# YushenLi807/WWW24-RAT

Hardware: AMD Instinct MI355X
Metric: training samples/sec at B=4096, K=10 retrieved, d=64; 1/2/4/8 MI355X (higher is better)
Workload: dtype f32; 1 GPU; synthetic_F20_V1M_K10_d64_B4096; fields=20, vocab_rows=1000000, retrieved=10, embedding_dim=64, batch_per_gpu=4096, global_batch=4096, heads=8, dim_head=10, depth=4, scale_dim=2, step=fwd+bwd+clip+adam, embedding_grad=atomic, sync_batch_norm=False, parallelism=dp1

## Files before the change

www24-rat_amd/csrc/attn.hip:

```cpp
#include "rat_device.h"
#include "../../include/rat_hip.h"

#include <cstdlib>
#include <initializer_list>

namespace {

constexpr int ATT_THREADS = 512;
constexpr int ATT_WAVES = ATT_THREADS / 64;
constexpr int ATT_ROWS = 64;
constexpr int ATT_MT = ATT_ROWS / 16;
constexpr int DH_MAX = 16;
constexpr int QSLOTS = 8;
constexpr int OSLOTS = 4;
constexpr int FAST_INNER = 80;
constexpr int fast_heads(int tdh) { return tdh > 0 ? FAST_INNER / tdh : 0; }
constexpr int CORE_UNROLL = 3;

struct AttnArgs {
    const float* x;
    const float* dy;
    float* y;
    const float* res;
    const float* add;
// ... 996 lines not shown
    RAT_REQUIRE(d <= 128, "embedding_dim > 128 is not supported by this kernel");
    RAT_REQUIRE(map->L >= 1 && map->L <= ATT_ROWS, "sequence length (K+1 or F+1) must be in [1, 64]");
    RAT_REQUIRE(map->nseq >= 1 && map->q_div >= 1, "bad seq map");
    const AttnGeom g(d, heads, dim_head);
    RAT_REQUIRE(g.fwd_smem() <= 160 * 1024, "heads*dim_head too large for the LDS tile (forward)");
    if (backward) {
        RAT_REQUIRE(g.bwd_smem(heads) <= 160 * 1024, "heads*dim_head too large for the LDS tile (backward)");
        RAT_REQUIRE((g.Q16 / 16) * (g.D16 / 16) <= QSLOTS * ATT_WAVES,
                    "3*heads*dim_head x embedding_dim exceeds the in-register dW_qkv accumulator budget");
        RAT_REQUIRE((g.D16 / 16) * (g.I16 / 16) <= OSLOTS * ATT_WAVES,
                    "embedding_dim x heads*dim_head exceeds the in-register dW_out accumulator budget");
    }
    return 0;
}

bool aligned16(const void* p) { return (reinterpret_cast<uintptr_t>(p) & 15) == 0; }

void fill_common(AttnArgs& a, const RatAttnParams* w, const RatSeqMap* map, int d, int heads, int dim_head,
                 float ln_eps) {
    a.ln_g = w->ln_g;
    a.ln_b = w->ln_b;
    a.w_qkv = w->w_qkv;
    a.w_out = w->w_out;
    a.b_out = w->b_out;
    a.nseq = map->nseq;
    a.q_div = map->q_div;
    a.hi_stride = map->hi_stride;
    a.lo_stride = map->lo_stride;
    a.pos_stride = map->pos_stride;
    a.L = map->L;
    a.nq = (map->queries > 0 && map->queries < map->L) ? map->queries : map->L;
    a.nsq_chunk = ATT_ROWS / map->L;
    a.nchunks = (map->nseq + a.nsq_chunk - 1) / a.nsq_chunk;
    a.d = d;
    a.heads = heads;
    a.dh = dim_head;
    a.eps = ln_eps;
    a.scale = 1.0f / sqrtf((float)dim_head);
    a.out_scale = 1.0f;
    const int I = heads * dim_head;
    a.vec_wqkv = (d % 4 == 0) && aligned16(w->w_qkv);
    a.vec_wout = (I % 4 == 0) && aligned16(w->w_out);
    a.prof = rat_prof_buffer();
}

bool aligned8(const void* p) { return (reinterpret_cast<uintptr_t>(p) & 7) == 0; }

int fast_dim(const AttnArgs& a, std::initializer_list<const void*> ptrs) {
    if (!((a.dh == 10 || a.dh == 20) && a.heads == fast_heads(a.dh)) || a.w_out == nullptr) return 0;
    for (const void* p : ptrs)
        if (p != nullptr && !aligned16(p)) return 0;
    if (!aligned16(a.w_qkv) || !aligned16(a.w_out)) return 0;
    return (a.d == 64 || a.d == 16) ? a.d : 0;
}

}

extern "C" int rat_attn_fwd(const float* x, float* y, float* o_save, float* lse_save, const RatAttnParams* w_host,
                            const RatSeqMap* map_host, int d, int heads, int dim_head, float ln_eps, void* stream) {
    return rat_attn_fwd_ex(x, x, y, o_save, lse_save, w_host, map_host, d, heads, dim_head, 0.f, 1.f, ln_eps, 0.f, 0, RAT_ARITH_F32,
                           nullptr, 0, stream);
}

static bool b3_dim(int d) { return d == B3_D || d == 40 || d == 48 || d == 56; }
static bool b3_geom(int d, int heads, int dim_head) {
    return (b3_dim(d) && heads == B3_H && dim_head == B3_DH) || (d == B3_D && heads == 4 && dim_head == 2 * B3_DH);
}
static bool b3_shape(int d, int heads, int dim_head, const RatAttnParams* w) {
    return b3_geom(d, heads, dim_head) && w->w_out != nullptr;
}
static bool b3_ph_fits(int L, int nsq_chunk, int heads = B3_H) { return (size_t)nsq_chunk * heads * L * L * 4 <= (size_t)3 * B3_XP; }
static int b3_matrix_core(int L) {
    const int k = rat_knob(RAT_KNOB_ATTN_BWD_CORE_MFMA);
    if (L > 48 || k == 0) return 0;
    if (L > 32) return (k == 1 || L >= 40) ? 13 : 0;
    return (k == 1 || L >= 28) ? (L > 16 ? 2 : 1) : 0;
}
static int b3_fwd_matrix_core(int L, int nq) {
    const int k = rat_knob(RAT_KNOB_ATTN_FWD_CORE_MFMA);
    if (L > 48 || nq < L || k == 3) return 0;
    if (k != 2 && !((L >= 28 && L <= 32) || L >= 40)) return 0;
    return L > 32 ? 3 : (L > 16 ? 2 : 1);
}
static bool b3_ph_enabled() {
    return rat_knob(RAT_KNOB_ATTN_BWD_PH) != 0;
}
static int b3_nvalid(int d) { return d == B3_D ? 0 : d; }
static bool b3_off32_ok(const RatSeqMap* m) {
    if (m->hi_stride < 0 || m->lo_stride < 0 || m->pos_stride < 0) return false;
    const int64_t qd = m->q_div, hi = (m->nseq - 1) / qd, lo = m->nseq - 1 < qd - 1 ? m->nseq - 1 : qd - 1;
    const double max_tok = (double)hi * (double)m->hi_stride + (double)lo * (double)m->lo_stride + (double)(m->L - 1) * (double)m->pos_stride;
    return (max_tok + 1.0) * (double)(B3_I * 4) < 4294967296.0;
}

extern "C" size_t rat_attn_fwd_workspace(int d, int heads, int dim_head) {
    return b3_geom(d, heads, dim_head) ? B3_W_QKV + B3_W_OUT : 0;
}

extern "C" size_t rat_attn_planes_bytes(int d, int heads, int dim_head) {
    return b3_geom(d, heads, dim_head) ? B3_W_BYTES : 0;
}
extern "C" int rat_attn_split_jobs(const RatAttnParams* w_host, int d, int heads, int dim_head, void* planes, RatSplitJob* jobs_out) {
    RAT_REQUIRE(w_host && jobs_out, "null pointer");
    if (!b3_shape(d, heads, dim_head, w_host) || planes == nullptr) return 0;
    RAT_REQUIRE(aligned16(planes) && w_host->w_qkv, "planes must be 16-byte aligned");
    char* ws = static_cast<char*>(planes);
    jobs_out[0] = RatSplitJob{w_host->w_qkv, ws, B3_Q3, d, d, 0, 0, 0};
    jobs_out[1] = RatSplitJob{w_host->w_out, ws + B3_W_QKV, B3_I, d, B3_I, 1, 0, 0};
    jobs_out[2] = RatSplitJob{w_host->w_qkv, ws + B3_W_QKV + B3_W_OUTT, B3_D, B3_Q3, d, 1, 0, b3_nvalid(d)};
    jobs_out[3] = RatSplitJob{w_host->w_out, ws + B3_W_QKV + B3_W_OUTT + B3_W_QKVT, B3_D, B3_I, B3_I, 0, 0, b3_nvalid(d)};
    return 4;
}

extern "C" int rat_attn_fwd_ex(const float* x, const float* res, float* y, float* o_save, float* lse_save,
                               const RatAttnParams* w_host, const RatSeqMap* map_host, int d, int heads, int dim_head,
                               float softmax_scale, float out_scale, float ln_eps, float dropout_p, uint64_t dropout_seed,
                               int arith, float* workspace, size_t workspace_bytes, void* stream) {
    if (check_dims(map_host, d, heads, dim_head, false)) return -1;
    RAT_REQUIRE(x && y && w_host && w_host->ln_g && w_host->ln_b && w_host->w_qkv, "null pointer");
    RAT_REQUIRE(w_host->w_out != nullptr || heads * dim_head == d, "missing w_out");
    AttnArgs a{};
    fill_common(a, w_host, map_host, d, heads, dim_head, ln_eps);
    if (softmax_scale > 0.f) a.scale = softmax_scale;
    a.out_scale = out_scale;
    a.res = res;
    a.x = x;
    a.y = y;
    a.o_save = o_save;
    a.lse_save = lse_save;
    a.vec_x = (d % 4 == 0) && aligned16(x) && aligned16(y) && aligned16(res);
    const AttnGeom g(d, heads, dim_head);
    const bool ct_shape = dim_head == 10 && ((d == 10 && (heads == 8 || heads == 2)) || (d == 16 && heads == 2));
    const size_t smem = g.fwd_smem() + (ct_shape ? ct_weight_floats(g) * sizeof(float) : 0);
    const int per_cu = (int)((160 * 1024) / smem) >= 2 ? 2 : 1;
    const unsigned blocks = (unsigned)(a.nchunks < rat_max_blocks() * per_cu ? a.nchunks : rat_max_blocks() * per_cu);
    RAT_REQUIRE(dropout_p >= 0.f && dropout_p < 1.f, "dropout_p must be in [0, 1)");
    if (dropout_p > 0.f && w_host->w_out != nullptr)
        a.drop = RatDrop{dropout_seed, (uint32_t)((double)dropout_p * 4294967296.0), 1.0f / (1.0f - dropout_p), w_host->drop_seed_dev};
    const int fast = fast_dim(a, {x, y, res, o_save, lse_save});
    const bool plain = res == x && out_scale == 1.0f && a.drop.threshold == 0;
    const bool have_planes = w_host->planes != nullptr && aligned16(w_host->planes);
    const bool dpad = d != B3_D && b3_dim(d) && heads == fast_heads(dim_head) && aligned16(x) && aligned16(y) && aligned16(res) &&
                      aligned16(o_save) && aligned16(lse_save) && aligned16(w_host->w_qkv) && aligned16(w_host->w_out);
    if (arith == RAT_ARITH_BF16X3 && (fast == 64 || dpad) && b3_shape(d, heads, dim_head, w_host) && b3_off32_ok(map_host) &&
        (have_planes || (workspace != nullptr && workspace_bytes >= B3_W_QKV + B3_W_OUT && aligned16(workspace)))) {
        const char* p_qkv;
        const char* p_out;
        if (have_planes) {
            p_qkv = static_cast<const char*>(w_host->planes);
            p_out = p_qkv + B3_W_QKV + B3_W_OUTT + B3_W_QKVT;
        } else {
            char* ws = reinterpret_cast<char*>(workspace);
            if (rat_launch_split_weights(w_host->w_qkv, B3_Q3, d, d, 0, ws, stream) ||
                rat_launch_split_weights(w_host->w_out, B3_D, B3_I, B3_I, 0, ws + B3_W_QKV, stream, 0, b3_nvalid(d))) return -1;
            p_qkv = ws;
            p_out = ws + B3_W_QKV;
        }
        Attn3W W{};
        W.qkv = RatWPlanes{reinterpret_cast<const rat_u4*>(p_qkv), 2};
        W.out = RatWPlanes{reinterpret_cast<const rat_u4*>(p_out), 3};
        const unsigned b3_blocks = (unsigned)(a.nchunks < rat_max_blocks() ? a.nchunks : rat_max_blocks());
        if (heads == 4) {
            RAT_LAUNCH((attn_fwd3_kernel<true, false, false, false, 0, 4>), b3_blocks, ATT_THREADS, b3_fwd_smem(), stream, a, W);
            return rat_check_launch("rat_attn_fwd (bf16x3, 4 heads)");
        }
        if (dpad) {
            if (plain && a.nq < a.L) RAT_LAUNCH((attn_fwd3_kernel<false, true, true>), b3_blocks, ATT_THREADS, b3_fwd_smem(), stream, a, W);
            else if (plain) RAT_LAUNCH((attn_fwd3_kernel<false, false, true>), b3_blocks, ATT_THREADS, b3_fwd_smem(), stream, a, W);
            else RAT_LAUNCH((attn_fwd3_kernel<true, false, true>), b3_blocks, ATT_THREADS, b3_fwd_smem(), stream, a, W);
        } else if (plain && a.nq < a.L) RAT_LAUNCH((attn_fwd3_kernel<false, true>), b3_blocks, ATT_THREADS, b3_fwd_smem(), stream, a, W);
        else if (plain && b3_fwd_matrix_core(a.L, a.nq) == 3)
            RAT_LAUNCH((attn_fwd3_kernel<false, false, false, false, 3>), b3_blocks, ATT_THREADS, b3_fwd_smem(), stream, a, W);
        else if (plain && b3_fwd_matrix_core(a.L, a.nq) == 2)
            RAT_LAUNCH((attn_fwd3_kernel<false, false, false, false, 2>), b3_blocks, ATT_THREADS, b3_fwd_smem(), stream, a, W);
        else if (plain && b3_fwd_matrix_core(a.L, a.nq) == 1)
            RAT_LAUNCH((attn_fwd3_kernel<false, false, false, false, 1>), b3_blocks, ATT_THREADS, b3_fwd_smem(), stream, a, W);
        else if (plain) RAT_LAUNCH((attn_fwd3_kernel<false>), b3_blocks, ATT_THREADS, b3_fwd_smem(), stream, a, W);
        else if (b3_fwd_matrix_core(a.L, a.L) == 3)
            RAT_LAUNCH((attn_fwd3_kernel<true, false, false, false, 3>), b3_blocks, ATT_THREADS, b3_fwd_smem(), stream, a, W);
        else if (b3_fwd_matrix_core(a.L, a.L) == 2)
            RAT_LAUNCH((attn_fwd3_kernel<true, false, false, false, 2>), b3_blocks, ATT_THREADS, b3_fwd_smem(), stream, a, W);
        else RAT_LAUNCH((attn_fwd3_kernel<true>), b3_blocks, ATT_THREADS, b3_fwd_smem(), stream, a, W);
        return rat_check_launch("rat_attn_fwd (bf16x3)");
    }
    const bool head_vec = aligned8(o_save);
    RAT_REQUIRE(head_vec || dim_head <= DH_MAX, "o_save must be 8-byte aligned for dim_head 20");
    if (!head_vec) RAT_LAUNCH((attn_fwd_kernel<0, 0>), blocks, ATT_THREADS, smem, stream, a);
    else if (fast == 64 && dim_head == 10 && plain) RAT_LAUNCH((attn_fwd_kernel<64, 10, false>), blocks, ATT_THREADS, smem, stream, a);
    else if (fast == 64 && dim_head == 10) RAT_LAUNCH((attn_fwd_kernel<64, 10>), blocks, ATT_THREADS, smem, stream, a);
    else if (fast == 16 && dim_head == 10) RAT_LAUNCH((attn_fwd_kernel<16, 10>), blocks, ATT_THREADS, smem, stream, a);
    else if (fast == 64 && dim_head == 20) RAT_LAUNCH((attn_fwd_kernel<64, 20>), blocks, ATT_THREADS, smem, stream, a);
    else if (dim_head == 20) RAT_LAUNCH((attn_fwd_kernel<0, 20>), blocks, ATT_THREADS, smem, stream, a);
    else if (dim_head == 10 && d == 10 && heads == 8) RAT_LAUNCH((attn_fwd_kernel<0, 10, true, 2, 8, 10>), blocks, ATT_THREADS, smem, stream, a);
    else if (dim_head == 10 && d == 10 && heads == 2) RAT_LAUNCH((attn_fwd_kernel<0, 10, true, 2, 2, 10>), blocks, ATT_THREADS, smem, stream, a);
    else if (dim_head == 10 && d == 16 && heads == 2) RAT_LAUNCH((attn_fwd_kernel<0, 10, true, 2, 2, 16>), blocks, ATT_THREADS, smem, stream, a);
    else if (dim_head == 10 && d <= 16) RAT_LAUNCH((attn_fwd_kernel<0, 10, true, 2>), blocks, ATT_THREADS, smem, stream, a);
    else if (dim_head == 10) RAT_LAUNCH((attn_fwd_kernel<0, 10>), blocks, ATT_THREADS, smem, stream, a);
    else RAT_LAUNCH((attn_fwd_kernel<0, 0>), blocks, ATT_THREADS, smem, stream, a);
    return rat_check_launch("rat_attn_fwd");
}

static int b3_groups(int d, int heads, int dim_head) {
    return (d == B3_D && dim_head == B3_DH && heads > B3_H && heads % B3_H == 0 && heads / B3_H <= 8) ? heads / B3_H : 0;
}
static int wide_heads(int dim_head) { return dim_head == WG_DH ? WG_H : (dim_head == 2 * WG_DH ? WG_H / 2 : 0); }
static int wide_groups(int d, int heads, int dim_head) {
    const int wh = wide_heads(dim_head);
    return (d >= 1 && d <= 16 && wh > 0 && heads > wh && heads % wh == 0 && heads / wh <= 8) ? heads / wh : 0;
}
extern "C" int rat_attn_groups_supported(int d, int heads, int dim_head) {
    if (b3_groups(d, heads, dim_head)) return 1;
    const int G = wide_groups(d, heads, dim_head);
    return G == 0 ? 0 : (G <= WG_MAXG ? 3 : 1);
}
extern "C" size_t rat_attn_groups_planes_bytes(int d, int heads, int dim_head) {
    return (size_t)b3_groups(d, heads, dim_head) * B3_GRP_PLANES;
}
extern "C" int rat_attn_groups_split_jobs(const RatAttnParams* w_host, int d, int heads, int dim_head, void* planes, RatSplitJob* jobs_out) {
    RAT_REQUIRE(w_host && jobs_out, "null pointer");
    const int G = b3_groups(d, heads, dim_head);
    if (G == 0 || planes == nullptr || w_host->w_out == nullptr) return 0;
    RAT_REQUIRE(aligned16(planes) && w_host->w_qkv, "planes must be 16-byte aligned");
    const int I = heads * dim_head;
    int n = 0;
    const int rows = (B3_I << 8) | (I << 20);
    for (int g = 0; g < G; ++g) {
        char* ws = static_cast<char*>(planes) + (size_t)g * B3_GRP_PLANES;
        const float* wq = w_host->w_qkv + (size_t)g * B3_I * d;
        const float* wo = w_host->w_out + (size_t)g * B3_I;
        jobs_out[n++] = RatSplitJob{wq, ws, B3_Q3, d, d, 0, rows, 0};
        jobs_out[n++] = RatSplitJob{wo, ws + B3_W_QKV, B3_I, d, I, 1, 0, 0};
        jobs_out[n++] = RatSplitJob{wq, ws + B3_W_QKV + B3_W_OUTT, B3_D, B3_Q3, d, 1, rows, 0};
        jobs_out[n++] = RatSplitJob{wo, ws + B3_W_QKV + B3_W_OUTT + B3_W_QKVT, B3_D, B3_I, I, 0, 0, 0};
    }
    return n;
}
extern "C" int rat_attn_fwd_groups(const float* x, const float* res, float* y, float* o_save, float* lse_save, int64_t ntok,
                                   const RatAttnParams* w_host, const void* planes, const RatSeqMap* map_host, int d, int heads,
                                   int dim_head, float softmax_scale, float out_scale, float ln_eps, float dropout_p,
                                   uint64_t dropout_seed, void* stream) {
    const int Gw = wide_groups(d, heads, dim_head);
    if (Gw > 0) {
        const int wh = wide_heads(dim_head);
        if (check_dims(map_host, d, wh, dim_head, false)) return -1;
        RAT_REQUIRE(x && y && w_host && w_host->ln_g && w_host->ln_b && w_host->w_qkv && w_host->w_out && w_host->b_out, "null pointer");
        RAT_REQUIRE((o_save == nullptr) == (lse_save == nullptr) && ntok > 0, "o_save and lse_save come together, [G][ntok][.]");
        AttnArgs a{};
        fill_common(a, w_host, map_host, d, wh, dim_head, ln_eps);
        a.vec_wout = ((heads * dim_head) % 4 == 0) && aligned16(w_host->w_out);
        a.vec_wqkv = (aligned8(x) && aligned16(w_host->w_out)) ? 1 : 0;
        if (softmax_scale > 0.f) a.scale = softmax_scale;
        a.out_scale = out_scale;
        a.res = res;
        a.x = x;
        a.y = y;
        a.o_save = o_save;
        a.lse_save = lse_save;
        a.groups = Gw;
        a.group_tok = ntok;
// ... 219 lines not shown
```

www24-rat_amd/csrc/attn_b3.h:

```cpp
constexpr int B3_D = 64, B3_I = 80, B3_Q3 = 240, B3_H = 8, B3_DH = 10;
constexpr int B3_LDQ = B3_Q3 + 4;
constexpr int B3_XP = 64 * 128;
constexpr int B3_OP = 64 * 160 + 64;
constexpr int B3_QP = 64 * 480;
typedef RatPlanes<128, 7, B3_XP> PlanesX;
typedef RatPlanes<160, 0, B3_OP> PlanesO;
typedef RatPlanes<480, 0, B3_QP> PlanesQ;

struct Attn3W {
    RatWPlanes qkv;
    RatWPlanes out;
    RatWPlanes outT;
    RatWPlanes qkvT;
};
constexpr size_t B3_W_QKV = (size_t)15 * 2 * 3 * 1024, B3_W_OUT = (size_t)4 * 3 * 3 * 1024, B3_W_OUTT = (size_t)5 * 2 * 3 * 1024,
                 B3_W_QKVT = (size_t)4 * 8 * 3 * 1024;
constexpr size_t B3_W_BYTES = B3_W_QKV + B3_W_OUT + B3_W_OUTT + B3_W_QKVT;

constexpr size_t B3_FWD_LSE = (size_t)3 * B3_XP + (size_t)64 * B3_LDQ * 4 + (size_t)3 * B3_OP + 2 * 64 * 8;
constexpr size_t B3_FWD_WOUT = B3_FWD_LSE + (size_t)64 * B3_H * 4;
constexpr size_t b3_fwd_smem() { return B3_FWD_WOUT + B3_W_OUT; }
constexpr size_t B3_GRP_PLANES = B3_W_BYTES;
static_assert(b3_fwd_smem() <= 160 * 1024, "LDS budget (forward)");
struct RatWPlanesLds {
// ... 133 lines not shown
    r = __builtin_amdgcn_permlane32_swap(rat_fbits(v), rat_fbits(v), false, false);
    return fmaxf(rat_bitsf(r[0]), rat_bitsf(r[1]));
#endif
}
__device__ __forceinline__ float b3m_rows_sum(float v) {
#ifdef RAT_EMU
    v += __shfl_xor(v, 16, 64);
    return v + __shfl_xor(v, 32, 64);
#else
    auto r = __builtin_amdgcn_permlane16_swap(rat_fbits(v), rat_fbits(v), false, false);
    v = rat_bitsf(r[0]) + rat_bitsf(r[1]);
    r = __builtin_amdgcn_permlane32_swap(rat_fbits(v), rat_fbits(v), false, false);
    return rat_bitsf(r[0]) + rat_bitsf(r[1]);
#endif
}
template <int NIT>
__device__ __forceinline__ void b3_fwd_core_mfma(float* qkv, float* lse_s, int L, int nsq, float scale) {
    const int w = rat_wave(), l = rat_lane(), g = l >> 4, m = l & 15;
    const float sl2 = scale * RAT_LOG2E;
    const int npairs = nsq * B3_H;
    for (int pair = w; pair < npairs; pair += ATT_WAVES) {
        const int h = pair % B3_H, sq = pair / B3_H;
        const int r0 = sq * L, cq = h * B3_DH, ck = B3_I + cq, cv = 2 * B3_I + cq;
        float ak[3][NIT], av[4][NIT];
#pragma unroll
        for (int jt = 0; jt < NIT; ++jt) {
#pragma unroll
            for (int ks = 0; ks < 3; ++ks) ak[ks][jt] = qkv[(size_t)(r0 + 16 * jt + m) * B3_LDQ + ck + 4 * ks + g];
#pragma unroll
            for (int r = 0; r < 4; ++r) av[r][jt] = qkv[(size_t)(r0 + 16 * jt + 4 * g + r) * B3_LDQ + cv + m];
        }
#pragma unroll
        for (int it = 0; it < NIT; ++it) {
            const int i0 = 16 * it;
            if (i0 >= L) break;
            const bool qok = i0 + m < L;
            float bq[3];
#pragma unroll
            for (int ks = 0; ks < 3; ++ks) bq[ks] = qkv[(size_t)(r0 + i0 + m) * B3_LDQ + cq + 4 * ks + g];
#pragma unroll
            for (int ks = 0; ks < 3; ++ks) bq[ks] = (4 * ks + g < B3_DH && qok) ? bq[ks] : 0.f;
            f32x4 st[NIT];
#pragma unroll
            for (int jt = 0; jt < NIT; ++jt) st[jt] = rat_zero4();
#pragma unroll
            for (int ks = 0; ks < 3; ++ks)
#pragma unroll
                for (int jt = 0; jt < NIT; ++jt) st[jt] = RAT_MFMA16(ak[ks][jt], bq[ks], st[jt]);
            float mx = -INFINITY;
#pragma unroll
            for (int jt = 0; jt < NIT; ++jt)
#pragma unroll
                for (int r = 0; r < 4; ++r) {
                    st[jt][r] = 16 * jt + 4 * g + r < L ? st[jt][r] * sl2 : -INFINITY;
                    mx = fmaxf(mx, st[jt][r]);
                }
            mx = b3m_rows_max(mx);
            float sum = 0.f;
#pragma unroll
            for (int jt = 0; jt < NIT; ++jt)
#pragma unroll
                for (int r = 0; r < 4; ++r) {
                    st[jt][r] = rat_exp2(st[jt][r] - mx);
                    sum += st[jt][r];
                }
            sum = b3m_rows_sum(sum);
            f32x4 ot = rat_zero4();
#pragma unroll
            for (int jt = 0; jt < NIT; ++jt)
#pragma unroll
                for (int r = 0; r < 4; ++r) ot = RAT_MFMA16(av[r][jt], st[jt][r], ot);
            const float inv = 1.0f / sum;
            if (qok) {
                float* op = qkv + (size_t)(r0 + i0 + m) * B3_LDQ + cq + 4 * g;
#pragma unroll
                for (int r = 0; r < 4; ++r)
                    if (4 * g + r < B3_DH) op[r] = ot[r] * inv;
                if (g == 0) lse_s[(r0 + i0 + m) * B3_H + h] = mx + rat_log2(sum);
            }
        }
    }
}

template <bool EX, bool QSUB = false, bool DPAD = false, bool GRP = false, int MCF = 0, int NH = B3_H>
__global__ void __launch_bounds__(ATT_THREADS) attn_fwd3_kernel(AttnArgs a, Attn3W W) {
    constexpr int NDH = B3_I / NH;
    static_assert(NH == B3_H || (NH == 4 && MCF == 0 && !GRP && !DPAD), "the matrix cores, the group loop and DPAD are written for 8 heads x 10");
    static_assert(!GRP || (EX && !QSUB && !DPAD), "the group loop is written for the general (EX) form at embedding_dim 64");
    static_assert(MCF == 0 || !QSUB, "the matrix core computes every query");
    RAT_DYN_SMEM(smem);
    const PlanesX xp{smem};
    float* qkv = reinterpret_cast<float*>(smem + 3 * B3_XP);
    const PlanesO op{smem + 3 * B3_XP + 64 * B3_LDQ * 4};
    int64_t* const rowtok0 = reinterpret_cast<int64_t*>(smem + 3 * B3_XP + 64 * B3_LDQ * 4 + 3 * B3_OP);
    float* ys = reinterpret_cast<float*>(smem);
    float* const lse_s = reinterpret_cast<float*>(smem + B3_FWD_LSE);
    constexpr int LDY = B3_D + 4;
    const int L = a.L;
    if (!GRP)
        for (int e = threadIdx.x; e < (int)(B3_W_OUT / 16); e += ATT_THREADS)
            reinterpret_cast<rat_u4*>(smem + B3_FWD_WOUT)[e] = W.out.base[e];
    const RatWPlanesLds wout_lds{smem + B3_FWD_WOUT, 3};

    for (int e = threadIdx.x; e < 3 * B3_OP / 4; e += ATT_THREADS) reinterpret_cast<float*>(op.base)[e] = 0.f;
    for (int e = threadIdx.x; e < 64 * (B3_LDQ - B3_Q3); e += ATT_THREADS) qkv[(e >> 2) * B3_LDQ + B3_Q3 + (e & 3)] = 0.f;
    const int dreal = DPAD ? a.d : B3_D;
    const bool colok = !DPAD || 8 * (int)(threadIdx.x & 7) < dreal;
    float gam[8], bet[8];
#pragma unroll
    for (int k = 0; k < 8; ++k) {
        gam[k] = colok ? a.ln_g[8 * (threadIdx.x & 7) + k] : 0.f;
        bet[k] = colok ? a.ln_b[8 * (threadIdx.x & 7) + k] : 0.f;
    }
    {
        int nsq0, rows0;
        map_rows(a, blockIdx.x, rowtok0, nsq0, rows0);
    }
    __syncthreads();
    RAT_PROF_DECL
    int parity = 0;
    for (int64_t chunk = blockIdx.x; chunk < a.nchunks; chunk += gridDim.x, parity ^= 1) {
        const int64_t* rowtok = rowtok0 + parity * ATT_ROWS;
        int nsq, rows;
        {
            const int64_t q0 = chunk * a.nsq_chunk;
            const int64_t left = a.nseq - q0;
            nsq = left < a.nsq_chunk ? (int)left : a.nsq_chunk;
            rows = nsq * a.L;
        }
        float4 x0, x1;
        b3_load_piece(a.x, rowtok, x0, x1, dreal, colok);
        b3_layer_norm_to_planes<DPAD>(rowtok[threadIdx.x >> 3] >= 0, x0, x1, a.eps, xp, gam, bet, nullptr, nullptr, dreal, colok);
        if (chunk + gridDim.x < a.nchunks) {
            int nsq1, rows1;
            map_rows(a, chunk + gridDim.x, (rowtok0 + (parity ^ 1) * ATT_ROWS), nsq1, rows1);
        }
        __syncthreads();
        RAT_PROF_MARK(0);
        float pf = 0.f;
        f32x4 yacc[2] = {rat_zero4(), rat_zero4()};
        const int ngroups = GRP ? a.groups : 1;
        for (int grp = 0; grp < ngroups; ++grp) {
        const RatWPlanes wq = GRP ? RatWPlanes{W.qkv.base + (size_t)grp * (B3_GRP_PLANES / 16), W.qkv.steps} : W.qkv;
        const RatWPlanes wo = GRP ? RatWPlanes{W.out.base + (size_t)grp * (B3_GRP_PLANES / 16), W.out.steps} : W.out;
        float* const o_save = (GRP && a.o_save != nullptr) ? a.o_save + (int64_t)grp * a.group_tok * B3_I : a.o_save;
        float* const lse_save = (GRP && a.lse_save != nullptr) ? a.lse_save + (int64_t)grp * a.group_tok * NH : a.lse_save;
        b3_gemm_rows<2>(xp, wq, B3_Q3 / 16, [&](int mt, int nt, const f32x4& acc) {
            const int col = rat_acc_col(nt);
#pragma unroll
            for (int r = 0; r < 4; ++r) qkv[(size_t)rat_acc_row(mt, r) * B3_LDQ + col] = acc[r];
        });
        __syncthreads();
        RAT_PROF_MARK(1);
        if ((int)threadIdx.x < ATT_ROWS * 2 && chunk + gridDim.x < a.nchunks && (!GRP || grp == ngroups - 1))
            pf = prefetch_lines_map((rowtok0 + (parity ^ 1) * ATT_ROWS), threadIdx.x, 2, a.x, dreal);
        typedef HeadVec<NDH> HV;
        const int nq = QSUB ? a.nq : L;
        const int ntasks = MCF ? 0 : nsq * NH * nq;
        const float sl2 = a.scale * RAT_LOG2E;
        if (MCF) b3_fwd_core_mfma<(MCF > 0 ? MCF : 1)>(qkv, lse_s, L, nsq, a.scale);
        for (int task = threadIdx.x; task < ntasks; task += ATT_THREADS) {
            const int i = task % nq;
            const int h = (task / nq) % NH;
            const int sq = task / (nq * NH);
            const int row_i = sq * L + i;
            float* qp = qkv + (size_t)row_i * B3_LDQ + h * NDH;
            HV q, o, kv;
            q.load(qp, NDH);
            o.zero();
            float m = -INFINITY, l = 0.f;
            const float* kbase = qkv + (size_t)(sq * L) * B3_LDQ + B3_I + h * NDH;
            int j = 0;
            for (; j + CORE_UNROLL <= L; j += CORE_UNROLL) {
                HV kk[CORE_UNROLL], vv[CORE_UNROLL];
#pragma unroll
                for (int u = 0; u < CORE_UNROLL; ++u) {
                    const float* kp = kbase + (size_t)(j + u) * B3_LDQ;
                    kk[u].load(kp, NDH);
                    vv[u].load(kp + B3_I, NDH);
                }
                float sc[CORE_UNROLL];
#pragma unroll
                for (int u = 0; u < CORE_UNROLL; ++u) sc[u] = q.dot(kk[u]) * sl2;
#pragma unroll
                for (int u = 0; u < CORE_UNROLL; ++u) {
                    const float mn = fmaxf(m, sc[u]);
                    const float corr = rat_exp2(m - mn);
                    const float p = rat_exp2(sc[u] - mn);
                    l = l * corr + p;
                    o.scale_axpy(corr, p, vv[u]);
                    m = mn;
                }
            }
            for (; j < L; ++j) {
                const float* kp = kbase + (size_t)j * B3_LDQ;
                kv.load(kp, NDH);
                const float sv = q.dot(kv) * sl2;
                const float mn = fmaxf(m, sv);
                const float corr = rat_exp2(m - mn);
                const float p = rat_exp2(sv - mn);
                l = l * corr + p;
// ... 770 lines not shown
```

www24-rat_amd/csrc/rat_common.hip:

```cpp
#include "rat_device.h"
#include <stdlib.h>
#include <vector>
#include "../../include/rat_hip.h"

static thread_local std::string g_last_error;

const char* rat_set_error(const std::string& msg) {
    g_last_error = msg;
    return g_last_error.c_str();
}
int rat_fail(const std::string& msg) {
    rat_set_error(msg);
    return -1;
}
int rat_check_launch(const char* what) {
    hipError_t e = hipGetLastError();
    if (e != hipSuccess) return rat_fail(std::string(what) + ": " + hipGetErrorString(e));
    return 0;
}

static int g_knobs[RAT_KNOB_COUNT];
static const char* const g_knob_names[RAT_KNOB_COUNT] = {"max_blocks", "attn_bwd_ph", "attn_fwd_core_mfma", "attn_bwd_core_mfma", "ffn_bwd_t3",
                                                         "sgemm_split_target"};
static const bool g_knobs_loaded = [] {
    auto env = [](const char* n) { const char* e = getenv(n); return e ? std::string(e) : std::string(); };
    const std::string mb = env("RAT_MAX_BLOCKS"), ph = env("RAT_ATTN_BWD_PH"), fc = env("RAT_ATTN_FWD_CORE"), bc = env("RAT_ATTN_BWD_CORE"),
                      ff = env("RAT_FFN_BWD"), st = env("RAT_SGEMM_SPLIT_TARGET");
    g_knobs[RAT_KNOB_MAX_BLOCKS] = mb.empty() ? 0 : atoi(mb.c_str());
    g_knobs[RAT_KNOB_ATTN_BWD_PH] = (ph.empty() || ph[0] != '0') ? 1 : 0;
    g_knobs[RAT_KNOB_ATTN_FWD_CORE_MFMA] = fc == "mfma" ? 1 : (fc == "mfma32" ? 2 : (fc == "valu" ? 3 : 0));
    g_knobs[RAT_KNOB_ATTN_BWD_CORE_MFMA] = bc == "mfma" ? 1 : (bc == "valu" ? 0 : -1);
    g_knobs[RAT_KNOB_FFN_BWD_T3] = ff.rfind("t3", 0) == 0 ? 1 : 0;
    g_knobs[RAT_KNOB_SGEMM_SPLIT_TARGET] = st.empty() ? 0 : (atoi(st.c_str()) > 0 ? atoi(st.c_str()) : 0);
    return true;
}();
int rat_knob(int which) { return g_knobs[which]; }
extern "C" int rat_debug_set_knob(const char* name, int value) {
    for (int i = 0; i < RAT_KNOB_COUNT; ++i)
        if (name != nullptr && std::string(name) == g_knob_names[i]) {
            const int old = g_knobs[i];
            g_knobs[i] = value;
            return old;
        }
    return -2147483647 - 1;
}
int rat_max_blocks() {
    const int n = g_knobs[RAT_KNOB_MAX_BLOCKS];
    return n > 0 && n < 256 ? n : 256;
}

static unsigned long long* g_prof = nullptr;
unsigned long long* rat_prof_buffer() { return g_prof; }
extern "C" void rat_debug_set_prof(void* device_u64x64) { g_prof = static_cast<unsigned long long*>(device_u64x64); }

extern "C" int rat_version(void) { return RAT_ABI_VERSION; }
extern "C" const char* rat_last_error(void) { return g_last_error.c_str(); }

struct RatReduceArgs {
    const float* slabs;
    int nslabs;
    int64_t stride;
    int nouts;
    float* out[8];
    int64_t off[8];
    int64_t size[8];
    int64_t first_block[9];
};

__global__ void __launch_bounds__(256) rat_reduce_slabs_kernel(RatReduceArgs r) {
    __shared__ float part[256];
    int o = 0;
    while (o + 1 < r.nouts && (int64_t)blockIdx.x >= r.first_block[o + 1]) ++o;
    const int lane_p = threadIdx.x & 63, quarter = threadIdx.x >> 6;
    const int64_t p = ((int64_t)blockIdx.x - r.first_block[o]) * 64 + lane_p;
    float s = 0.f;
    if (p < r.size[o]) {
        const int per = (r.nslabs + 3) / 4;
        const int w0 = quarter * per, w1 = (w0 + per < r.nslabs) ? w0 + per : r.nslabs;
        const float* src = r.slabs + r.off[o] + p;
        int w = w0;
        for (; w + 8 <= w1; w += 8) {
            float v[8];
#pragma unroll
            for (int k = 0; k < 8; ++k) v[k] = src[(int64_t)(w + k) * r.stride];
#pragma unroll
            for (int k = 0; k < 8; ++k) s += v[k];
        }
        for (; w < w1; ++w) s += src[(int64_t)w * r.stride];
    }
    part[threadIdx.x] = s;
    __syncthreads();
    if (quarter == 0 && p < r.size[o]) r.out[o][p] = ((part[lane_p] + part[64 + lane_p]) + part[128 + lane_p]) + part[192 + lane_p];
}

struct RatReduceEntry {
    const float* src;
    float* out;
    int64_t size, stride;
    int nslabs, first_block;
};
constexpr int RAT_REDUCE_BATCH = 80;
struct RatReduceTable {
    RatReduceEntry e[RAT_REDUCE_BATCH];
    int n, blocks;
};
static thread_local bool g_defer = false;
static thread_local std::vector<RatReduceEntry> g_deferred;

__global__ void __launch_bounds__(256) rat_reduce_slabs_batch_kernel(RatReduceTable t) {
    __shared__ float4 part4[256];
    float* part = reinterpret_cast<float*>(part4);
    int o = 0;
    auto first = [&](int i) { const int f = t.e[i].first_block; return f < 0 ? -f - 1 : f; };
    while (o + 1 < t.n && (int)blockIdx.x >= first(o + 1)) ++o;
    const RatReduceEntry& r = t.e[o];
    const bool vec = r.first_block < 0;
// ... 219 lines not shown
```

www24-rat_amd/csrc/rat_device.h:

```cpp
#pragma once

#include <stdint.h>
#include <stddef.h>

#ifdef RAT_EMU
#include "hip_emu.h"
#define RAT_MFMA16(a, b, c) emu_mfma_f32_16x16x4f32((a), (b), (c))
#define RAT_MFMA4(a, b, c) emu_mfma_f32_4x4x1f32((a), (b), (c))
#else
#include <hip/hip_runtime.h>
typedef float f32x4 __attribute__((vector_size(16)));
#define RAT_MFMA16(a, b, c) __builtin_amdgcn_mfma_f32_16x16x4f32((a), (b), (c), 0, 0, 0)
#define RAT_MFMA4(a, b, c) __builtin_amdgcn_mfma_f32_4x4x1f32((a), (b), (c), 0, 0, 0)
#define RAT_LAUNCH(kernel, grid, block, smem, stream, ...) \
    hipLaunchKernelGGL(kernel, dim3(grid), dim3(block), (smem), (hipStream_t)(stream), __VA_ARGS__)
#define RAT_DYN_SMEM(name) extern __shared__ __attribute__((aligned(16))) char name[]
#endif

#include <string>

#if defined(RAT_PROF) && !defined(RAT_EMU)
#define RAT_PROF_DECL unsigned long long prof_t0 = clock64(); unsigned long long prof_acc[12] = {0, 0, 0, 0, 0, 0, 0, 0, 0, 0, 0, 0};
#define RAT_PROF_MARK(i) do { const unsigned long long prof_t = clock64(); prof_acc[i] += prof_t - prof_t0; prof_t0 = prof_t; } while (0)
#define RAT_PROF_FLUSH(ptr, base) do { if (threadIdx.x == 0 && (ptr) != nullptr) for (int pi = 0; pi < 12; ++pi) atomicAdd((ptr) + (base) + pi, prof_acc[pi]); } while (0)
#define RAT_TRACE(ptr, on, slot) do { if ((ptr) != nullptr && (on) && blockIdx.x == 0 && (threadIdx.x & 63) == 0) (ptr)[256 + (threadIdx.x >> 6) * 32 + (slot)] = clock64(); } while (0)
#else
#define RAT_PROF_DECL
#define RAT_PROF_MARK(i) do { } while (0)
#define RAT_PROF_FLUSH(ptr, base) do { } while (0)
#define RAT_TRACE(ptr, on, slot) do { } while (0)
#endif
#ifdef RAT_EMU
#define RAT_WAVE_FENCE() emu::wave_sync()
#else
#define RAT_WAVE_FENCE() do { __builtin_amdgcn_fence(__ATOMIC_ACQ_REL, "wavefront"); __builtin_amdgcn_wave_barrier(); } while (0)
#endif
unsigned long long* rat_prof_buffer();

const char* rat_set_error(const std::string& msg);
int rat_fail(const std::string& msg);
int rat_check_launch(const char* what);
enum { RAT_KNOB_MAX_BLOCKS, RAT_KNOB_ATTN_BWD_PH, RAT_KNOB_ATTN_FWD_CORE_MFMA, RAT_KNOB_ATTN_BWD_CORE_MFMA, RAT_KNOB_FFN_BWD_T3,
       RAT_KNOB_SGEMM_SPLIT_TARGET, RAT_KNOB_COUNT };
int rat_knob(int which);
int rat_max_blocks();

#define RAT_REQUIRE(cond, msg)                  \
    do {                                        \
        if (!(cond)) return rat_fail(std::string(__func__) + ": " + (msg)); \
    } while (0)

static inline int rat_round_up(int v, int m) { return (v + m - 1) / m * m; }

#define RAT_WAVE 64
#ifdef RAT_EMU
#define RAT_SCHED_FENCE() do { } while (0)
#define RAT_SCHED_MFMA_VALU(n, v) do { } while (0)
#else
#define RAT_SCHED_FENCE() __builtin_amdgcn_sched_barrier(0)
#define RAT_SCHED_MFMA_VALU(n, v)                                   \
    do {                                                            \
        _Pragma("unroll") for (int sgb_i = 0; sgb_i < (n); ++sgb_i) { \
            __builtin_amdgcn_sched_group_barrier(0x008, 1, 0);      \
            __builtin_amdgcn_sched_group_barrier(0x002, (v), 0);    \
        }                                                           \
    } while (0)
#endif

__device__ __forceinline__ int rat_lane() { return threadIdx.x & 63; }
#ifdef RAT_EMU
__device__ __forceinline__ int rat_wave() { return threadIdx.x >> 6; }
#else
__device__ __forceinline__ int rat_wave() { return __builtin_amdgcn_readfirstlane((int)(threadIdx.x >> 6)); }
#endif

__device__ __forceinline__ float4 rat_consume4(const float4& src) {
#ifdef RAT_EMU
    return src;
#else
    float4 d;
    asm volatile("v_mov_b32 %0, %4\n\tv_mov_b32 %1, %5\n\tv_mov_b32 %2, %6\n\tv_mov_b32 %3, %7"
                 : "=&v"(d.x), "=&v"(d.y), "=&v"(d.z), "=&v"(d.w)
                 : "v"(src.x), "v"(src.y), "v"(src.z), "v"(src.w));
    return d;
#endif
}

__device__ __forceinline__ uint32_t rat_hash32(uint64_t seed, uint64_t i) {
    uint64_t z = seed + 0x9E3779B97F4A7C15ull * (i + 1);
    z = (z ^ (z >> 30)) * 0xBF58476D1CE4E5B9ull;
    z = (z ^ (z >> 27)) * 0x94D049BB133111EBull;
    z = z ^ (z >> 31);
    return (uint32_t)(z >> 32);
}
struct RatDrop {
    uint64_t seed;
    uint32_t threshold;
    float scale;
    const uint64_t* seed_dev;
    __device__ __forceinline__ uint64_t the_seed() const { return seed_dev != nullptr ? *seed_dev : seed; }
    __device__ __forceinline__ float apply(float v, int64_t idx) const {
        return threshold == 0 ? v : (rat_hash32(the_seed(), (uint64_t)idx) >= threshold ? v * scale : 0.f);
    }
};

__device__ __forceinline__ void rat_st4_stream(float* p, const float4& v) {
#ifdef RAT_EMU
    *reinterpret_cast<float4*>(p) = v;
#else
    const f32x4 t = {v.x, v.y, v.z, v.w};
    __builtin_nontemporal_store(t, reinterpret_cast<f32x4*>(p));
#endif
}
__device__ __forceinline__ float4 rat_ld4_stream(const float* p) {
#ifdef RAT_EMU
    return *reinterpret_cast<const float4*>(p);
#else
    const f32x4 t = __builtin_nontemporal_load(reinterpret_cast<const f32x4*>(p));
    return make_float4(t[0], t[1], t[2], t[3]);
#endif
}

__device__ __forceinline__ f32x4 rat_zero4() {
    f32x4 z = {0.f, 0.f, 0.f, 0.f};
    return z;
}
// ... 509 lines not shown
```

Baseline: 223,800 samples/s.

## Add rotated attention forward loop overlapping next chunk QKV GEMM with softmax core

Adds a software-pipelined variant of the plain 8x10-head bf16x3 attention forward kernel. The next chunk's QKV projection MFMAs are interleaved with the current chunk's VALU online-softmax core using sched_group_barrier hints, and the layer norm and row mapping run two chunks ahead through a triple-buffered rowtok scheme. It is enabled by default through a new env knob and applies only when the plain path is not already routed to an MFMA attention core. The aim is to hide matrix-core GEMM latency behind VALU attention work, at the cost of more registers held in accumulators and extra LDS for the third row-token buffer.

```diff
diff --git a/www24-rat_amd/csrc/attn.hip b/www24-rat_amd/csrc/attn.hip
--- a/www24-rat_amd/csrc/attn.hip
+++ b/www24-rat_amd/csrc/attn.hip
@@ -1102,6 +1102,7 @@
     if (k != 2 && !((L >= 28 && L <= 32) || L >= 40)) return 0;
     return L > 32 ? 3 : (L > 16 ? 2 : 1);
 }
+static bool b3_fwd_rotated_enabled() { return rat_knob(RAT_KNOB_ATTN_FWD_ROTATED) != 0; }
 static bool b3_ph_enabled() {
     return rat_knob(RAT_KNOB_ATTN_BWD_PH) != 0;
 }
@@ -1195,6 +1196,8 @@
             RAT_LAUNCH((attn_fwd3_kernel<false, false, false, false, 2>), b3_blocks, ATT_THREADS, b3_fwd_smem(), stream, a, W);
         else if (plain && b3_fwd_matrix_core(a.L, a.nq) == 1)
             RAT_LAUNCH((attn_fwd3_kernel<false, false, false, false, 1>), b3_blocks, ATT_THREADS, b3_fwd_smem(), stream, a, W);
+        else if (plain && b3_fwd_rotated_enabled())
+            RAT_LAUNCH((attn_fwd3_kernel<false, false, false, false, 0, B3_H, true>), b3_blocks, ATT_THREADS, b3_fwd_rot_smem(), stream, a, W);
         else if (plain) RAT_LAUNCH((attn_fwd3_kernel<false>), b3_blocks, ATT_THREADS, b3_fwd_smem(), stream, a, W);
         else if (b3_fwd_matrix_core(a.L, a.L) == 3)
             RAT_LAUNCH((attn_fwd3_kernel<true, false, false, false, 3>), b3_blocks, ATT_THREADS, b3_fwd_smem(), stream, a, W);
diff --git a/www24-rat_amd/csrc/attn_b3.h b/www24-rat_amd/csrc/attn_b3.h
--- a/www24-rat_amd/csrc/attn_b3.h
+++ b/www24-rat_amd/csrc/attn_b3.h
@@ -239,9 +239,247 @@
     }
 }
 
-template <bool EX, bool QSUB = false, bool DPAD = false, bool GRP = false, int MCF = 0, int NH = B3_H>
+constexpr size_t b3_fwd_rot_smem() { return b3_fwd_smem() + (size_t)ATT_ROWS * 8; }
+static_assert(b3_fwd_rot_smem() <= 160 * 1024, "LDS budget (rotated forward)");
+template <int UPG, bool GEMM>
+__device__ __forceinline__ void b3_fwd_core_rot(float* qkv, float* lse_s, const PlanesX& xp, const RatWPlanes& wq, int L, int nsq, float sl2,
+                                                f32x4 (&acc)[4][2]) {
+    typedef HeadVec<B3_DH> HV;
+    const int ntasks = nsq * B3_H * L;
+    const bool live = (int)threadIdx.x < ntasks;
+    const int task = live ? (int)threadIdx.x : 0;
+    const int i = task % L;
+    const int h = (task / L) % B3_H;
+    const int sq = task / (L * B3_H);
+    const int row_i = sq * L + i;
+    float* qp = qkv + (size_t)row_i * B3_LDQ + h * B3_DH;
+    HV q, o, kv;
+    q.load(qp, B3_DH);
+    o.zero();
+    float m = -INFINITY, l = 0.f;
+    const float* kbase = qkv + (size_t)(sq * L) * B3_LDQ + B3_I + h * B3_DH;
+    auto keys = [&](int j) {
+        HV kk[CORE_UNROLL], vv[CORE_UNROLL];
+#pragma unroll
+        for (int u = 0; u < CORE_UNROLL; ++u) {
+            const float* kp = kbase + (size_t)(j + u) * B3_LDQ;
+            kk[u].load(kp, B3_DH);
+            vv[u].load(kp + B3_I, B3_DH);
+        }
+        float sc[CORE_UNROLL];
+#pragma unroll
+        for (int u = 0; u < CORE_UNROLL; ++u) sc[u] = q.dot(kk[u]) * sl2;
+#pragma unroll
+        for (int u = 0; u < CORE_UNROLL; ++u) {
+            const float mn = fmaxf(m, sc[u]);
+            const float corr = rat_exp2(m - mn);
+            const float p = rat_exp2(sc[u] - mn);
+            l = l * corr + p;
+            o.scale_axpy(corr, p, vv[u]);
+            m = mn;
+        }
+    };
+    int j = 0;
+    if (GEMM) {
+        constexpr int NU = 8, VPM = 8 / UPG;
+        const int w = rat_wave(), mt0 = 2 * (w >> 2), ntb = w & 3;
+        auto bfrag = [&](int u) { return wq(ntb + 4 * (u & 3) < B3_Q3 / 16 ? ntb + 4 * (u & 3) : ntb, u >> 2); };
+        RatB3 af[2], b = bfrag(0);
+#pragma unroll
+        for (int t = 0; t < 4; ++t) acc[t][0] = acc[t][1] = rat_zero4();
+#pragma unroll
+        for (int st = 0; st < NU / UPG; ++st) {
+            const bool loaded = j + CORE_UNROLL <= L;
+            auto units = [&]() {
+#pragma unroll
+                for (int k = 0; k < UPG; ++k) {
+                    const int u = st * UPG + k;
+                    if ((u & 3) == 0) {
+                        af[0] = xp.row_frag(mt0, u >> 2);
+                        af[1] = xp.row_frag(mt0 + 1, u >> 2);
+                    }
+                    const RatB3 bn = bfrag(u + 1 < NU ? u + 1 : u);
+                    rat_mfma3_block<2>(acc[u & 3], af, b);
+                    b = bn;
+                }
+            };
+            if (loaded) {
+                units();
+                keys(j);
+                j += CORE_UNROLL;
+#ifndef RAT_EMU
+#pragma unroll
+                for (int k = 0; k < 12 * UPG; ++k) {
+                    __builtin_amdgcn_sched_group_barrier(0x8, 1, 0);
+                    __builtin_amdgcn_sched_group_barrier(0x2, VPM, 0);
+                }
+#endif
+            } else {
+                units();
+            }
+        }
+    }
+    for (; j + CORE_UNROLL <= L; j += CORE_UNROLL) keys(j);
+    for (; j < L; ++j) {
+        const float* kp = kbase + (size_t)j * B3_LDQ;
+        kv.load(kp, B3_DH);
+        const float sv = q.dot(kv) * sl2;
+        const float mn = fmaxf(m, sv);
+        const float corr = rat_exp2(m - mn);
+        const float p = rat_exp2(sv - mn);
+        l = l * corr + p;
+        kv.load(kp + B3_I, B3_DH);
+        o.scale_axpy(corr, p, kv);
+        m = mn;
+    }
+    if (live) {
+        const float inv = 1.0f / l;
+        o.store(qp, B3_DH, inv);
+        lse_s[row_i * B3_H + h] = m + rat_log2(l);
+    }
+}
+
+__device__ __forceinline__ void b3_fwd_rotated(const AttnArgs& a, const Attn3W& W, char* smem) {
+    const PlanesX xp{smem};
+    float* qkv = reinterpret_cast<float*>(smem + 3 * B3_XP);
+    const PlanesO op{smem + 3 * B3_XP + 64 * B3_LDQ * 4};
+    int64_t* const rowtok0 = reinterpret_cast<int64_t*>(smem + 3 * B3_XP + 64 * B3_LDQ * 4 + 3 * B3_OP);
+    int64_t* const rowtok2 = reinterpret_cast<int64_t*>(smem + b3_fwd_smem());
+    float* ys = reinterpret_cast<float*>(smem);
+    float* const lse_s = reinterpret_cast<float*>(smem + B3_FWD_LSE);
+    constexpr int LDY = B3_D + 4;
+    const RatWPlanesLds wout_lds{smem + B3_FWD_WOUT, 3};
+    const int L = a.L;
+    const int64_t G = gridDim.x;
+    int64_t chunk = blockIdx.x;
+    if (chunk >= a.nchunks) return;
+    auto rt = [&](int k) { return k < 2 ? rowtok0 + k * ATT_ROWS : rowtok2; };
+    auto tile_epi = [&](int mt, int nt, const f32x4& acc) {
+        const int col = rat_acc_col(nt);
+#pragma unroll
+        for (int r = 0; r < 4; ++r) qkv[(size_t)rat_acc_row(mt, r) * B3_LDQ + col] = acc[r];
+    };
+    auto ln_chunk = [&](const int64_t* rowtok) {
+        float4 x0, x1;
+        b3_load_piece(a.x, rowtok, x0, x1);
+        float gam[8], bet[8];
+#pragma unroll
+        for (int k = 0; k < 8; ++k) {
+            gam[k] = a.ln_g[8 * (threadIdx.x & 7) + k];
+            bet[k] = a.ln_b[8 * (threadIdx.x & 7) + k];
+        }
+        b3_layer_norm_to_planes<false>(rowtok[threadIdx.x >> 3] >= 0, x0, x1, a.eps, xp, gam, bet, nullptr, nullptr);
+    };
+    RAT_PROF_DECL
+    ln_chunk(rt(0));
+    {
+        int nsq1, rows1;
+        if (chunk + G < a.nchunks) map_rows(a, chunk + G, rt(1), nsq1, rows1);
+        if (chunk + 2 * G < a.nchunks) map_rows(a, chunk + 2 * G, rt(2), nsq1, rows1);
+    }
+    __syncthreads();
+    b3_gemm_rows<2>(xp, W.qkv, B3_Q3 / 16, tile_epi);
+    __syncthreads();
+    if (chunk + G < a.nchunks) ln_chunk(rt(1));
+    __syncthreads();
+    RAT_PROF_MARK(0);
+    const float sl2 = a.scale * RAT_LOG2E;
+    int k0 = 0;
+    for (;;) {
+        const bool next1 = chunk + G < a.nchunks, next2 = chunk + 2 * G < a.nchunks;
+        const int k1 = k0 == 2 ? 0 : k0 + 1, k2 = k1 == 2 ? 0 : k1 + 1;
+        const int64_t* rowtok = rt(k0);
+        int nsq;
+        {
+            const int64_t left = a.nseq - chunk * a.nsq_chunk;
+            nsq = left < a.nsq_chunk ? (int)left : a.nsq_chunk;
+        }
+        float pf = 0.f;
+        if ((int)threadIdx.x < ATT_ROWS * 2 && next2) pf = prefetch_lines_map(rt(k2), threadIdx.x, 2, a.x, B3_D);
+        f32x4 acc[4][2];
+        if (next1) {
+            if (L >= 6 * CORE_UNROLL) b3_fwd_core_rot<1, true>(qkv, lse_s, xp, W.qkv, L, nsq, sl2, acc);
+            else if (L >= 3 * CORE_UNROLL) b3_fwd_core_rot<2, true>(qkv, lse_s, xp, W.qkv, L, nsq, sl2, acc);
+            else b3_fwd_core_rot<4, true>(qkv, lse_s, xp, W.qkv, L, nsq, sl2, acc);
+        } else {
+            b3_fwd_core_rot<1, false>(qkv, lse_s, xp, W.qkv, L, nsq, sl2, acc);
+        }
+        __syncthreads();
+        RAT_PROF_MARK(2);
+        for (int e = threadIdx.x; e < ATT_ROWS * (B3_I / 8); e += ATT_THREADS) {
+            const int r = e / (B3_I / 8), o8 = e - r * (B3_I / 8);
+            const float* src = qkv + (size_t)r * B3_LDQ + 8 * o8;
+            const float4 v0 = *reinterpret_cast<const float4*>(src), v1 = *reinterpret_cast<const float4*>(src + 4);
+            rat_u4 h, m, l;
+            rat_split8(v0, v1, h, m, l);
+            op.store(r, o8, h, m, l);
+            const int64_t tok = rowtok[r];
+            if (a.o_save != nullptr && tok >= 0) {
+                rat_st4_stream(a.o_save + tok * B3_I + 8 * o8, v0);
+                rat_st4_stream(a.o_save + tok * B3_I + 8 * o8 + 4, v1);
+            }
+        }
+        if (a.lse_save != nullptr && (int)threadIdx.x < (B3_H / 4) * ATT_ROWS) {
+            const int r = threadIdx.x / (B3_H / 4), part = threadIdx.x % (B3_H / 4);
+            const int64_t tok = rowtok[r];
+            if (tok >= 0) rat_st4_stream(a.lse_save + tok * B3_H + 4 * part, *reinterpret_cast<const float4*>(lse_s + r * B3_H + 4 * part));
+        }
+        __syncthreads();
+        RAT_PROF_MARK(3);
+        float4 x0, x1;
+        b3_load_piece(a.x, rowtok, x0, x1);
+        b3_gemm_rows<3>(op, wout_lds, B3_D / 16, [&](int mt, int nt, const f32x4& c) {
+            const int col = rat_acc_col(nt);
+            const float bias = a.b_out[col];
+#pragma unroll
+            for (int r = 0; r < 4; ++r) ys[(size_t)rat_acc_row(mt, r) * LDY + col] = c[r] + bias;
+        });
+        __syncthreads();
+        RAT_PROF_MARK(4);
+        if (next1) {
+            const int w = rat_wave(), mt0 = 2 * (w >> 2);
+#pragma unroll
+            for (int t = 0; t < 4; ++t) {
+                const int nt = (w & 3) + 4 * t;
+                if (nt < B3_Q3 / 16) {
+                    tile_epi(mt0, nt, acc[t][0]);
+                    tile_epi(mt0 + 1, nt, acc[t][1]);
+                }
+            }
+        }
+        {
+            const int r = threadIdx.x >> 3, sb = threadIdx.x & 7;
+            const int64_t tok = rowtok[r];
+            if (tok >= 0) {
+                const float4 t0 = *reinterpret_cast<const float4*>(ys + (size_t)r * LDY + 8 * sb);
+                const float4 t1 = *reinterpret_cast<const float4*>(ys + (size_t)r * LDY + 8 * sb + 4);
+                *reinterpret_cast<float4*>(a.y + tok * B3_D + 8 * sb) = make_float4(t0.x + x0.x, t0.y + x0.y, t0.z + x0.z, t0.w + x0.w);
+                *reinterpret_cast<float4*>(a.y + tok * B3_D + 8 * sb + 4) = make_float4(t1.x + x1.x, t1.y + x1.y, t1.z + x1.z, t1.w + x1.w);
+            }
+        }
+        __syncthreads();
+#ifndef RAT_EMU
+        asm volatile("" ::"v"(pf));
+#endif
+        RAT_PROF_MARK(5);
+        if (!next1) break;
+        if (next2) ln_chunk(rt(k2));
+        if (chunk + 3 * G < a.nchunks) {
+            int nsq3, rows3;
+            map_rows(a, chunk + 3 * G, rt(k0), nsq3, rows3);
+        }
+        __syncthreads();
+        RAT_PROF_MARK(0);
+        chunk += G;
+        k0 = k1;
+    }
+    RAT_PROF_FLUSH(a.prof, 48);
+}
+
+template <bool EX, bool QSUB = false, bool DPAD = false, bool GRP = false, int MCF = 0, int NH = B3_H, bool ROT = false>
 __global__ void __launch_bounds__(ATT_THREADS) attn_fwd3_kernel(AttnArgs a, Attn3W W) {
     constexpr int NDH = B3_I / NH;
+    static_assert(!ROT || (!EX && !QSUB && !DPAD && !GRP && MCF == 0 && NH == B3_H), "the rotated loop is written for the plain 8 x 10 form, VALU core");
     static_assert(NH == B3_H || (NH == 4 && MCF == 0 && !GRP && !DPAD), "the matrix cores, the group loop and DPAD are written for 8 heads x 10");
     static_assert(!GRP || (EX && !QSUB && !DPAD), "the group loop is written for the general (EX) form at embedding_dim 64");
     static_assert(MCF == 0 || !QSUB, "the matrix core computes every query");
@@ -274,6 +512,10 @@
         map_rows(a, blockIdx.x, rowtok0, nsq0, rows0);
     }
     __syncthreads();
+    if (ROT) {
+        b3_fwd_rotated(a, W, smem);
+        return;
+    }
     RAT_PROF_DECL
     int parity = 0;
     for (int64_t chunk = blockIdx.x; chunk < a.nchunks; chunk += gridDim.x, parity ^= 1) {
diff --git a/www24-rat_amd/csrc/rat_common.hip b/www24-rat_amd/csrc/rat_common.hip
--- a/www24-rat_amd/csrc/rat_common.hip
+++ b/www24-rat_amd/csrc/rat_common.hip
@@ -21,17 +21,18 @@
 
 static int g_knobs[RAT_KNOB_COUNT];
 static const char* const g_knob_names[RAT_KNOB_COUNT] = {"max_blocks", "attn_bwd_ph", "attn_fwd_core_mfma", "attn_bwd_core_mfma", "ffn_bwd_t3",
-                                                         "sgemm_split_target"};
+                                                         "sgemm_split_target", "attn_fwd_rotated"};
 static const bool g_knobs_loaded = [] {
     auto env = [](const char* n) { const char* e = getenv(n); return e ? std::string(e) : std::string(); };
     const std::string mb = env("RAT_MAX_BLOCKS"), ph = env("RAT_ATTN_BWD_PH"), fc = env("RAT_ATTN_FWD_CORE"), bc = env("RAT_ATTN_BWD_CORE"),
-                      ff = env("RAT_FFN_BWD"), st = env("RAT_SGEMM_SPLIT_TARGET");
+                      ff = env("RAT_FFN_BWD"), st = env("RAT_SGEMM_SPLIT_TARGET"), ro = env("RAT_ATTN_FWD_ROT");
     g_knobs[RAT_KNOB_MAX_BLOCKS] = mb.empty() ? 0 : atoi(mb.c_str());
     g_knobs[RAT_KNOB_ATTN_BWD_PH] = (ph.empty() || ph[0] != '0') ? 1 : 0;
     g_knobs[RAT_KNOB_ATTN_FWD_CORE_MFMA] = fc == "mfma" ? 1 : (fc == "mfma32" ? 2 : (fc == "valu" ? 3 : 0));
     g_knobs[RAT_KNOB_ATTN_BWD_CORE_MFMA] = bc == "mfma" ? 1 : (bc == "valu" ? 0 : -1);
     g_knobs[RAT_KNOB_FFN_BWD_T3] = ff.rfind("t3", 0) == 0 ? 1 : 0;
     g_knobs[RAT_KNOB_SGEMM_SPLIT_TARGET] = st.empty() ? 0 : (atoi(st.c_str()) > 0 ? atoi(st.c_str()) : 0);
+    g_knobs[RAT_KNOB_ATTN_FWD_ROTATED] = (ro.empty() || ro[0] != '0') ? 1 : 0;
     return true;
 }();
 int rat_knob(int which) { return g_knobs[which]; }
diff --git a/www24-rat_amd/csrc/rat_device.h b/www24-rat_amd/csrc/rat_device.h
--- a/www24-rat_amd/csrc/rat_device.h
+++ b/www24-rat_amd/csrc/rat_device.h
@@ -41,7 +41,7 @@
 int rat_fail(const std::string& msg);
 int rat_check_launch(const char* what);
 enum { RAT_KNOB_MAX_BLOCKS, RAT_KNOB_ATTN_BWD_PH, RAT_KNOB_ATTN_FWD_CORE_MFMA, RAT_KNOB_ATTN_BWD_CORE_MFMA, RAT_KNOB_FFN_BWD_T3,
-       RAT_KNOB_SGEMM_SPLIT_TARGET, RAT_KNOB_COUNT };
+       RAT_KNOB_SGEMM_SPLIT_TARGET, RAT_KNOB_ATTN_FWD_ROTATED, RAT_KNOB_COUNT };
 int rat_knob(int which);
 int rat_max_blocks();
 
```

Result: slower. 220,300 samples/s (-1.6%).
